# zju3dv/LoG

Hardware: NVIDIA B200
Metric: gaussians_per_s_fwd_bwd (higher is better)
Workload: dtype f32

## Files before the change

log_b200/csrc/lgr_blend.cu:

```cuda
#include "lgr_common.cuh"
#include "lgr_prof.cuh"

namespace lgr {

constexpr int BLEND_THREADS = TILE_PIX;
#ifndef LGR_FWD_MIN_CTAS
#define LGR_FWD_MIN_CTAS 5
#endif
#ifndef LGR_BWD_MIN_CTAS
#define LGR_BWD_MIN_CTAS 4
#endif
constexpr int BATCH = 256;
constexpr unsigned FULL = 0xffffffffu;

struct SubTile {
  int x, y;
  bool inside;
};

__device__ __forceinline__ SubTile make_subtile(const View& v, int tile, int lane, int warp) {
  SubTile s;
  const int tx = tile % v.gx, ty = v.row0 + tile / v.gx;
  const int sx = tx * TILE + (warp & 1) * 8, sy = ty * TILE + (warp >> 1) * 4;
  s.x = sx + (lane & 7); s.y = sy + (lane >> 3);
  s.inside = s.x < v.W && s.y < v.H;
  return s;
}

__device__ __forceinline__ unsigned subtile_bits(const float4 r0, const float4 r1, float tx0, float ty0) {
  const float xlo = r0.x - r1.z, xhi = r0.x + r1.z, ylo = r0.y - r1.w, yhi = r0.y + r1.w;
  unsigned xm = 0u, m = 0u;
  if (xhi >= tx0 && xlo <= tx0 + 7.0f) xm |= 1u;
  if (xhi >= tx0 + 8.0f && xlo <= tx0 + 15.0f) xm |= 2u;
#pragma unroll
  for (int r = 0; r < 4; r++)
    if (yhi >= ty0 + 4.0f * r && ylo <= ty0 + 4.0f * r + 3.0f) m |= xm << (2 * r);
  return m;
}

__device__ __forceinline__ float eval_power2(const float4 r0, const float con_z, float dx, float dy) {
  const float q = __fmaf_rn(r0.z, __fmul_rn(dx, dx), __fmul_rn(con_z, __fmul_rn(dy, dy)));
  return __fmaf_rn(-0.5f, q, -__fmul_rn(r0.w, __fmul_rn(dx, dy)));
}
__device__ __forceinline__ float ex2_approx(float x) {
  float y;
  asm("ex2.approx.ftz.f32 %0, %1;" : "=f"(y) : "f"(x));
  return y;
}
__device__ __forceinline__ float eval_alpha(float opacity, float G) { return fminf(ALPHA_MAX, __fmul_rn(opacity, G)); }

__device__ __forceinline__ uint32_t smem_u32(const void* p) { return (uint32_t)__cvta_generic_to_shared(p); }
__device__ __forceinline__ float4 lds_f4(uint32_t addr) {
  float4 v;
  asm volatile("ld.shared.v4.f32 {%0, %1, %2, %3}, [%4];" : "=f"(v.x), "=f"(v.y), "=f"(v.z), "=f"(v.w) : "r"(addr));
  return v;
}
__device__ __forceinline__ float2 lds_f2(uint32_t addr) {
  float2 v;
  asm volatile("ld.shared.v2.f32 {%0, %1}, [%2];" : "=f"(v.x), "=f"(v.y) : "r"(addr));
  return v;
}
__device__ __forceinline__ uint32_t pin_reg(uint32_t v) {
  asm volatile("" : "+r"(v));
  return v;
}
__device__ __forceinline__ void red_shared_max_u32(uint32_t addr, unsigned v) {
  asm volatile("red.shared.max.u32 [%0], %1;" ::"r"(addr), "r"(v) : "memory");
}
__device__ __forceinline__ void red_shared_add_f32(uint32_t addr, float v) {
  asm volatile("red.shared.add.f32 [%0], %1;" ::"r"(addr), "f"(v) : "memory");
}
__device__ __forceinline__ void sts_f32(uint32_t addr, float v) {
  asm volatile("st.shared.f32 [%0], %1;" ::"r"(addr), "f"(v) : "memory");
}
__device__ __forceinline__ float rcp_approx(float x) {
  float y;
  asm("rcp.approx.ftz.f32 %0, %1;" : "=f"(y) : "f"(x));
  return y;
}
__device__ __forceinline__ void prefetch_l2(const float* p) {
  asm volatile("prefetch.global.L2 [%0];" ::"l"(p));
}
__device__ __forceinline__ float tf32_lo(float x) { return x - __uint_as_float(__float_as_uint(x) & 0xffffe000u); }
__device__ __forceinline__ void ldsm_x4(uint32_t addr, uint32_t& r0, uint32_t& r1, uint32_t& r2, uint32_t& r3) {
  asm volatile("ldmatrix.sync.aligned.m8n8.x4.shared.b16 {%0, %1, %2, %3}, [%4];"
               : "=r"(r0), "=r"(r1), "=r"(r2), "=r"(r3) : "r"(addr));
}
__device__ __forceinline__ void mma_tf32(float& d0, float& d1, float& d2, float& d3, uint32_t a0, uint32_t a1, uint32_t a2,
                                         uint32_t a3, uint32_t b0, uint32_t b1) {
  asm volatile("mma.sync.aligned.m16n8k8.row.col.f32.tf32.tf32.f32 {%0, %1, %2, %3}, {%4, %5, %6, %7}, {%8, %9}, {%0, %1, %2, %3};"
               : "+f"(d0), "+f"(d1), "+f"(d2), "+f"(d3) : "r"(a0), "r"(a1), "r"(a2), "r"(a3), "r"(b0), "r"(b1));
}

__device__ __forceinline__ void stage_splat(float4* s_rec, unsigned char* s_bits, int slot, const float* __restrict__ splat,
                                            int id, float tx0, float ty0, const uint8_t* __restrict__ recorded = nullptr) {
  const float* rec = splat + (int64_t)id * LGR_SPLAT_FLOATS;
  const float4 r0 = ldg4(rec), r1 = ldg4(rec + 4);
  float4 r2 = ldg4(rec + 8);
  r2.w = __int_as_float(id);
  s_rec[3 * slot] = r0; s_rec[3 * slot + 1] = r1; s_rec[3 * slot + 2] = r2;
  s_bits[slot] = recorded ? *recorded : (unsigned char)subtile_bits(r0, r1, tx0, ty0);
}

template <bool AUX, bool REC>
__global__ void __launch_bounds__(BLEND_THREADS, LGR_FWD_MIN_CTAS)
blend_fwd_kernel(View v, const int32_t* __restrict__ tile_start, const int32_t* __restrict__ sorted_ids,
                 const float* __restrict__ splat, float* __restrict__ image, float* __restrict__ final_T,
                 int32_t* __restrict__ n_contrib, int32_t* __restrict__ pid_pixel, float* __restrict__ pw_pixel,
                 unsigned* __restrict__ point_weight_bits, int32_t* __restrict__ point_count) {
  __shared__ float4 s_rec[BATCH * 3];
  __shared__ unsigned s_w[AUX ? BATCH : 1];
  __shared__ unsigned char s_bits[BATCH];
  __shared__ unsigned s_cb[REC ? (BLEND_THREADS / 32) * (BATCH / 32) : 1];
  const int tile = blockIdx.x, tid = threadIdx.x, lane = tid & 31, warp = tid >> 5;
  const SubTile st = make_subtile(v, tile, lane, warp);
  const float pxf = (float)st.x, pyf = (float)st.y;
  const float tx0 = (float)((tile % v.gx) * TILE), ty0 = (float)((v.row0 + tile / v.gx) * TILE);
  const int beg = tile_start[tile], len = tile_start[tile + 1] - beg;
  const uint32_t s_w_addr = smem_u32(s_w);
  const uint32_t s_rec_addr = pin_reg(smem_u32(s_rec));

  float T = 1.0f, C0 = 0.f, C1 = 0.f, C2 = 0.f, wmax = 0.f;
  int last = 0, wid = -1;
  int done = st.inside ? 0 : 1;
  int id_next = tid < len ? sorted_ids[beg + tid] : -1;

  int base = 0, cnt = min(BATCH, len);
  auto stage = [&]() {
    if (tid < cnt) stage_splat(s_rec, s_bits, tid, splat, id_next, tx0, ty0);
    else s_bits[tid] = 0;
    if (AUX) s_w[tid] = 0u;
    id_next = base + BATCH + tid < len ? sorted_ids[beg + base + BATCH + tid] : -1;
    if (id_next >= 0) prefetch_l2(splat + (int64_t)id_next * LGR_SPLAT_FLOATS);
  };
  if (len > 0) stage();
  while (base < len) {
    __syncthreads();
    if (REC) {
      if (lane < BATCH / 32) s_cb[warp * (BATCH / 32) + lane] = 0u;
      __syncwarp();
    }
    if (!__all_sync(FULL, done)) {
      for (int c0 = 0; c0 < cnt; c0 += 32) {
        const int e_l = c0 + lane;
        unsigned mask = __ballot_sync(FULL, (s_bits[e_l] >> warp) & 1u);
        unsigned own_w = 0u;
        unsigned took = 0u;
        while (mask) {
          const int jA = __ffs(mask) - 1;
          mask &= mask - 1;
          const bool two = mask != 0u;
          const int jB = two ? __ffs(mask) - 1 : jA;
          mask &= mask - 1;
          const uint32_t recA = s_rec_addr + 48u * (uint32_t)(c0 + jA), recB = s_rec_addr + 48u * (uint32_t)(c0 + jB);
          const float4 r0A = lds_f4(recA), r0B = lds_f4(recB);
          const float2 r1A = lds_f2(recA + 16u), r1B = lds_f2(recB + 16u);
          const float dxA = __fsub_rn(r0A.x, pxf), dyA = __fsub_rn(r0A.y, pyf);
          const float dxB = __fsub_rn(r0B.x, pxf), dyB = __fsub_rn(r0B.y, pyf);
          const float powerA = eval_power2(r0A, r1A.x, dxA, dyA), powerB = eval_power2(r0B, r1B.x, dxB, dyB);
          const float alphaA = eval_alpha(r1A.y, ex2_approx(powerA)), alphaB = eval_alpha(r1B.y, ex2_approx(powerB));
          float wA = 0.f, wB = 0.f;
          if (!done && powerA <= 0.0f && alphaA >= ALPHA_MIN) {
            const float test_T = __fmul_rn(T, __fsub_rn(1.0f, alphaA));
            if (test_T < T_STOP) done = 1;
            else {
              wA = alphaA * T;
              const float4 r2 = lds_f4(recA + 32u);
              C0 = fmaf(r2.x, wA, C0); C1 = fmaf(r2.y, wA, C1); C2 = fmaf(r2.z, wA, C2);
              T = test_T;
              last = base + c0 + jA + 1;
              if (AUX && wA > wmax) { wmax = wA; wid = __float_as_int(r2.w); }
            }
          }
          if (two && !done && powerB <= 0.0f && alphaB >= ALPHA_MIN) {
            const float test_T = __fmul_rn(T, __fsub_rn(1.0f, alphaB));
            if (test_T < T_STOP) done = 1;
            else {
              wB = alphaB * T;
              const float4 r2 = lds_f4(recB + 32u);
              C0 = fmaf(r2.x, wB, C0); C1 = fmaf(r2.y, wB, C1); C2 = fmaf(r2.z, wB, C2);
              T = test_T;
              last = base + c0 + jB + 1;
              if (AUX && wB > wmax) { wmax = wB; wid = __float_as_int(r2.w); }
            }
          }
          if (AUX) {
            const unsigned mA = __reduce_max_sync(FULL, __float_as_uint(wA));
            const unsigned mB = __reduce_max_sync(FULL, __float_as_uint(wB));
            if (lane == jA) own_w = mA;
            if (two && lane == jB) own_w = mB;
          } else if (REC) {
            if (__any_sync(FULL, wA != 0.f)) took |= 1u << jA;
            if (__any_sync(FULL, wB != 0.f)) took |= 1u << jB;
          }
        }
        if (AUX && REC) took = __ballot_sync(FULL, own_w != 0u);
        if (REC && lane == 0) s_cb[warp * (BATCH / 32) + (c0 >> 5)] = took;
        if (AUX && own_w) red_shared_max_u32(s_w_addr + 4u * e_l, own_w);
        if (__all_sync(FULL, done)) break;
      }
    }
    const int all_done = __syncthreads_and(done);
    if (AUX && tid < cnt && s_w[tid]) atomicMax(point_weight_bits + __float_as_int(s_rec[3 * tid + 2].w), s_w[tid]);
    if (REC && tid < cnt) {
      unsigned byte = 0u;
#pragma unroll
      for (int w = 0; w < BLEND_THREADS / 32; w++) byte |= ((s_cb[w * (BATCH / 32) + (tid >> 5)] >> (tid & 31)) & 1u) << w;
      v.contrib[beg + base + tid] = (uint8_t)byte;
    }
    base += BATCH;
    if (all_done || base >= len) break;
    cnt = min(BATCH, len - base);
    stage();
  }
  if (st.inside) {
    const int64_t pix = (int64_t)st.y * v.W + st.x, HW = (int64_t)v.H * v.W;
    image[pix] = C0 + T * __ldg(v.bg);
    image[HW + pix] = C1 + T * __ldg(v.bg + 1);
    image[2 * HW + pix] = C2 + T * __ldg(v.bg + 2);
    final_T[pix] = T;
    n_contrib[pix] = last;
    if (AUX) {
      pid_pixel[pix] = (v.pid_map && wid >= 0) ? v.pid_map[wid] : wid; pw_pixel[pix] = wmax;
      if (point_count && wid >= 0) atomicAdd(point_count + wid, 1);
    }
  }
}

constexpr int HITS = 8;
constexpr int XROW = 36;
constexpr int BWD_SMEM = BATCH * 48 + BATCH * 36 + (BLEND_THREADS / 32) * (2 * HITS * XROW + 192 + 192) * 4 + BATCH;

template <bool REC>
__global__ void __launch_bounds__(BLEND_THREADS, LGR_BWD_MIN_CTAS)
blend_bwd_kernel(View v, const int32_t* __restrict__ tile_start, const int32_t* __restrict__ sorted_ids,
                 const float* __restrict__ splat, const float* __restrict__ image,
                 const float* __restrict__ dL_dimage, float* __restrict__ dsplat) {
  extern __shared__ float4 smem_f4[];
  float4* s_rec = smem_f4;
  float* s_g = reinterpret_cast<float*>(s_rec + BATCH * 3);
  float* s_x = s_g + BATCH * 9;
  float* s_cw = s_x + (BLEND_THREADS / 32) * 2 * HITS * XROW;
  float* s_mw = s_cw + (BLEND_THREADS / 32) * 192;
  unsigned char* s_bits = reinterpret_cast<unsigned char*>(s_mw + (BLEND_THREADS / 32) * 192);
  const int tile = blockIdx.x, tid = threadIdx.x, lane = tid & 31, warp = tid >> 5;
  const SubTile st = make_subtile(v, tile, lane, warp);
  const float pxf = (float)st.x, pyf = (float)st.y;
  const float tx0 = (float)((tile % v.gx) * TILE), ty0 = (float)((v.row0 + tile / v.gx) * TILE);
  const int beg = tile_start[tile], len = tile_start[tile + 1] - beg;
  const uint32_t s_g_addr = pin_reg(smem_u32(s_g));
  const uint32_t s_rec_addr = pin_reg(smem_u32(s_rec));
  const uint32_t xg_addr = pin_reg(smem_u32(s_x) + (uint32_t)warp * (2 * HITS * XROW * 4));
  const uint32_t xlane_addr = pin_reg(xg_addr + 4u * (uint32_t)lane);
  const uint32_t xrow = pin_reg(xg_addr + (uint32_t)(lane & 7) * (XROW * 4) + (uint32_t)((lane >> 3) & 1) * (HITS * XROW * 4) +
                                (uint32_t)(lane >> 4) * 16u);
  const float tcx = tx0 + 7.5f, tcy = ty0 + 7.5f;
  const int g = lane >> 2, t = lane & 3;

  float Rd = 0.f, dp0 = 0.f, dp1 = 0.f, dp2 = 0.f;
  int last = 0;
  if (st.inside) {
    const int64_t pix = (int64_t)st.y * v.W + st.x, HW = (int64_t)v.H * v.W;
    dp0 = dL_dimage[pix]; dp1 = dL_dimage[HW + pix]; dp2 = dL_dimage[2 * HW + pix];
    Rd = image[pix] * dp0 + image[HW + pix] * dp1 + image[2 * HW + pix] * dp2;
    if (REC) last = v.last_contrib[pix];
  }
  const uint32_t mw_addr = pin_reg(smem_u32(s_mw) + (uint32_t)warp * (192 * 4) + (uint32_t)((min(g, 5) * 4 + t) * 32));
  for (int k = lane; k < 192; k += 32) {
    const int which = k & 1, s_ = (k >> 1) & 3, t_ = (k >> 3) & 3, g_ = k >> 5;
    const float u = (float)((warp & 1) * 8 + t_ + 4 * which) - 7.5f, vv = (float)((warp >> 1) * 4 + s_) - 7.5f;
    const float f = g_ == 0 ? 1.f : g_ == 1 ? u : g_ == 2 ? vv : g_ == 3 ? u * u : g_ == 4 ? u * vv : vv * vv;
    s_mw[warp * 192 + k] = f;
  }
  const uint32_t cw_addr = pin_reg(smem_u32(s_cw) + (uint32_t)warp * (192 * 4) + (uint32_t)((min(g, 2) * 4 + t) * 64));
  {
    float* cw = s_cw + warp * 192;
    const int col = lane & 7, s = lane >> 3, tt = col & 3, which = col >> 2;
    const float dpc[3] = {dp0, dp1, dp2};
#pragma unroll
    for (int c = 0; c < 3; c++) {
      cw[((c * 4 + tt) * 4 + s) * 4 + which] = dpc[c];
      cw[((c * 4 + tt) * 4 + s) * 4 + 2 + which] = tf32_lo(dpc[c]);
    }
  }
  __syncwarp();

  float T = 1.0f;
  int done = st.inside ? (REC ? (last == 0) : 0) : 1;
  int id_next = tid < len ? sorted_ids[beg + tid] : -1;

  int base = 0, cnt = min(BATCH, len);
  auto stage = [&]() {
    if (tid < cnt) {
      stage_splat(s_rec, s_bits, tid, splat, id_next, tx0, ty0, REC ? v.contrib + beg + base + tid : nullptr);
#pragma unroll
      for (int k = 0; k < 9; k++) s_g[tid * 9 + k] = 0.f;
    } else {
      s_bits[tid] = 0;
    }
    id_next = base + BATCH + tid < len ? sorted_ids[beg + base + BATCH + tid] : -1;
    if (id_next >= 0) prefetch_l2(splat + (int64_t)id_next * LGR_SPLAT_FLOATS);
  };
  if (len > 0) stage();
  while (base < len) {
    __syncthreads();
    if (!__all_sync(FULL, done)) {
      int c0 = -32, pend = 0, my_e = 0;
      unsigned mask = 0u;
      bool fin = false;
      while (true) {
        if (mask == 0u) {
          do {
            c0 += 32;
            fin = c0 >= cnt || __all_sync(FULL, done);
            if (fin) break;
            mask = __ballot_sync(FULL, (s_bits[c0 + lane] >> warp) & 1u);
          } while (mask == 0u);
        }
        if (!fin) {
          const int jA = __ffs(mask) - 1;
          mask &= mask - 1;
          const bool two = mask != 0u;
          const int jB = two ? __ffs(mask) - 1 : jA;
          mask &= mask - 1;
          const int eA = c0 + jA, eB = c0 + jB;
          const uint32_t recA = s_rec_addr + 48u * (uint32_t)eA, recB = s_rec_addr + 48u * (uint32_t)eB;
          const float4 r0A = lds_f4(recA), r0B = lds_f4(recB);
          const float2 r1A = lds_f2(recA + 16u), r1B = lds_f2(recB + 16u);
          const float dxA = __fsub_rn(r0A.x, pxf), dyA = __fsub_rn(r0A.y, pyf);
          const float dxB = __fsub_rn(r0B.x, pxf), dyB = __fsub_rn(r0B.y, pyf);
          const float powerA = eval_power2(r0A, r1A.x, dxA, dyA), powerB = eval_power2(r0B, r1B.x, dxB, dyB);
          const float GA = ex2_approx(powerA), GB = ex2_approx(powerB);
          const float alphaA = eval_alpha(r1A.y, GA), alphaB = eval_alpha(r1B.y, GB);
          const float omA = __fsub_rn(1.0f, alphaA), omB = __fsub_rn(1.0f, alphaB);
          bool cA = false, cB = false;
          const float TA = T;
          float TB;
          if (REC) {
            cA = !done && powerA <= 0.0f && alphaA >= ALPHA_MIN;
            if (cA) T = __fmul_rn(T, omA);
            done = (base + eA + 1 >= last);
            TB = T;
            cB = two && !done && powerB <= 0.0f && alphaB >= ALPHA_MIN;
            if (cB) T = __fmul_rn(T, omB);
            if (two) done = (base + eB + 1 >= last);
          } else {
            if (!done && powerA <= 0.0f && alphaA >= ALPHA_MIN) {
              const float tt = __fmul_rn(T, omA);
              if (tt < T_STOP) done = 1; else { cA = true; T = tt; }
            }
            TB = T;
            if (two && !done && powerB <= 0.0f && alphaB >= ALPHA_MIN) {
              const float tt = __fmul_rn(T, omB);
              if (tt < T_STOP) done = 1; else { cB = true; T = tt; }
            }
          }
          const bool anyA = __any_sync(FULL, cA), anyB = __any_sync(FULL, cB);
          if (anyA) {
            float wG = 0.f, w = 0.f;
            if (cA) {
              const float4 r2 = lds_f4(recA + 32u);
              w = alphaA * TA;
              const float cdot = r2.x * dp0 + r2.y * dp1 + r2.z * dp2;
              Rd = fmaf(-cdot, w, Rd);
              const float dL_dalpha = cdot * TA - Rd * rcp_approx(omA);
              wG = r1A.y * dL_dalpha * GA;
            }
            const uint32_t row = xlane_addr + (uint32_t)pend * (XROW * 4);
            sts_f32(row, wG); sts_f32(row + HITS * XROW * 4, w);
            if (lane == pend) my_e = eA;
            pend++;
          }
          if (anyB) {
            float wG = 0.f, w = 0.f;
            if (cB) {
              const float4 r2 = lds_f4(recB + 32u);
              w = alphaB * TB;
              const float cdot = r2.x * dp0 + r2.y * dp1 + r2.z * dp2;
              Rd = fmaf(-cdot, w, Rd);
              const float dL_dalpha = cdot * TB - Rd * rcp_approx(omB);
              wG = r1B.y * dL_dalpha * GB;
            }
            const uint32_t row = xlane_addr + (uint32_t)pend * (XROW * 4);
            sts_f32(row, wG); sts_f32(row + HITS * XROW * 4, w);
            if (lane == pend) my_e = eB;
            pend++;
          }
        }
        if (pend >= HITS - 1 || (fin && pend > 0)) {
          __syncwarp();
          float d0 = 0.f, d1 = 0.f, z0 = 0.f, z1 = 0.f, y0 = 0.f, y1 = 0.f, d2 = 0.f, d3 = 0.f;
#pragma unroll
          for (int s = 0; s < 4; s++) {
            uint32_t a0, a1, a2, a3;
            ldsm_x4(xrow + 32u * s, a0, a1, a2, a3);
            const uint32_t l0 = __float_as_uint(tf32_lo(__uint_as_float(a0))), l1 = __float_as_uint(tf32_lo(__uint_as_float(a1)));
            const uint32_t l2 = __float_as_uint(tf32_lo(__uint_as_float(a2))), l3 = __float_as_uint(tf32_lo(__uint_as_float(a3)));
            float2 bm = make_float2(0.f, 0.f);
            float4 bc = make_float4(0.f, 0.f, 0.f, 0.f);
            if (g < 6) bm = lds_f2(mw_addr + 8u * s);
            if (g < 3) bc = lds_f4(cw_addr + 16u * s);
            mma_tf32(d0, d1, z0, z1, a0, a1, a2, a3, __float_as_uint(bm.x), __float_as_uint(bm.y));
            mma_tf32(y0, y1, d2, d3, a0, a1, a2, a3, __float_as_uint(bc.x), __float_as_uint(bc.y));
            mma_tf32(d0, d1, z0, z1, l0, l1, l2, l3, __float_as_uint(bm.x), __float_as_uint(bm.y));
            mma_tf32(y0, y1, d2, d3, l0, l1, l2, l3, __float_as_uint(bc.x), __float_as_uint(bc.y));
            mma_tf32(y0, y1, d2, d3, a0, a1, a2, a3, __float_as_uint(bc.z), __float_as_uint(bc.w));
          }
          const uint32_t acc = s_g_addr + 36u * (uint32_t)__shfl_sync(FULL, my_e, g);
          if (g < pend) {
            if (t < 3) { red_shared_add_f32(acc + 8u * t, d0); red_shared_add_f32(acc + 8u * t + 4u, d1); }
            if (t < 2) red_shared_add_f32(acc + 24u + 8u * t, d2);
            if (t == 0) red_shared_add_f32(acc + 28u, d3);
          }
          __syncwarp();
          pend = 0;
        }
        if (fin) break;
      }
    }
    const int all_done = __syncthreads_and(done);
    if (tid < cnt) {
      const float* m = s_g + tid * 9;
      const float M00 = m[0], M10 = m[1], M01 = m[2], M20 = m[3], M11 = m[4], M02 = m[5];
      const bool nz = (M00 != 0.f) | (M10 != 0.f) | (M01 != 0.f) | (M20 != 0.f) | (M11 != 0.f) | (M02 != 0.f) |
                      (m[6] != 0.f) | (m[7] != 0.f) | (m[8] != 0.f);
      if (nz) {
        const float4 r0 = s_rec[3 * tid];
        const float2 r1 = *reinterpret_cast<const float2*>(&s_rec[3 * tid + 1]);
        const int id = __float_as_int(s_rec[3 * tid + 2].w);
        const float X = r0.x - tcx, Y = r0.y - tcy;
        const float Sx = fmaf(X, M00, -M10), Sy = fmaf(Y, M00, -M01);
        const float Sxx = fmaf(X, fmaf(X, M00, -2.f * M10), M20);
        const float Syy = fmaf(Y, fmaf(Y, M00, -2.f * M01), M02);
        const float Sxy = fmaf(X, fmaf(Y, M00, -M01), fmaf(-Y, M10, M11));
        float4 a, b;
        a.x = -(r0.z * Sx + r0.w * Sy);
        a.y = -(r1.x * Sy + r0.w * Sx);
        a.z = -0.5f * Sxx;
        a.w = -Sxy;
        b.x = -0.5f * Syy;
        b.y = M00 / r1.y;
        b.z = m[6]; b.w = m[7];
        float4* dst = reinterpret_cast<float4*>(dsplat + (int64_t)id * LGR_GRAD_FLOATS);
        atomicAdd(dst, a);
        atomicAdd(dst + 1, b);
        atomicAdd(reinterpret_cast<float*>(dst + 2), m[8]);
      }
    }
    base += BATCH;
    if (all_done || base >= len) break;
    cnt = min(BATCH, len - base);
    stage();
  }
}

int launch_blend_fwd(const View& v, const int32_t* tile_start, const int32_t* sorted_ids, const float* splat,
                     float* image, float* final_T, int32_t* n_contrib, int32_t* pid_pixel, float* pw_pixel,
                     float* point_weight, int32_t* point_count, cudaStream_t st) {
  const int ntiles = v.gx * (v.row1 - v.row0);
  if (ntiles <= 0) return 0;
  ProfScope ps(K_BLEND_FWD, st);
  unsigned* pwb = reinterpret_cast<unsigned*>(point_weight);
  const bool rec = v.contrib != nullptr;
  if (v.want_aux && rec)
    blend_fwd_kernel<true, true><<<ntiles, BLEND_THREADS, 0, st>>>(v, tile_start, sorted_ids, splat, image, final_T, n_contrib, pid_pixel, pw_pixel, pwb, point_count);
  else if (v.want_aux)
    blend_fwd_kernel<true, false><<<ntiles, BLEND_THREADS, 0, st>>>(v, tile_start, sorted_ids, splat, image, final_T, n_contrib, pid_pixel, pw_pixel, pwb, point_count);
  else if (rec)
    blend_fwd_kernel<false, true><<<ntiles, BLEND_THREADS, 0, st>>>(v, tile_start, sorted_ids, splat, image, final_T, n_contrib, pid_pixel, pw_pixel, pwb, point_count);
  else
    blend_fwd_kernel<false, false><<<ntiles, BLEND_THREADS, 0, st>>>(v, tile_start, sorted_ids, splat, image, final_T, n_contrib, pid_pixel, pw_pixel, pwb, point_count);
  LGR_CHECK_LAUNCH();
  return 0;
}

int launch_blend_bwd(const View& v, const int32_t* tile_start, const int32_t* sorted_ids, const float* splat,
                     const float* image, const float* dL_dimage, float* dsplat, cudaStream_t st) {
  const int ntiles = v.gx * (v.row1 - v.row0);
  if (ntiles <= 0) return 0;
  const bool rec = v.contrib != nullptr && v.last_contrib != nullptr;
  cudaError_t e = rec ? cudaFuncSetAttribute(blend_bwd_kernel<true>, cudaFuncAttributeMaxDynamicSharedMemorySize, BWD_SMEM)
                      : cudaFuncSetAttribute(blend_bwd_kernel<false>, cudaFuncAttributeMaxDynamicSharedMemorySize, BWD_SMEM);
  if (e != cudaSuccess) return (int)e;
  ProfScope ps(K_BLEND_BWD, st);
  if (rec) blend_bwd_kernel<true><<<ntiles, BLEND_THREADS, BWD_SMEM, st>>>(v, tile_start, sorted_ids, splat, image, dL_dimage, dsplat);
  else blend_bwd_kernel<false><<<ntiles, BLEND_THREADS, BWD_SMEM, st>>>(v, tile_start, sorted_ids, splat, image, dL_dimage, dsplat);
  LGR_CHECK_LAUNCH();
  return 0;
}

}
```

profiles/sass_census.py:

```python
import collections
import os
import re
import subprocess

ROOT = os.path.dirname(os.path.dirname(os.path.abspath(__file__)))
LIB = os.path.join(ROOT, 'log_b200', '_lib', 'liblog_b200_raster.so')
PATS = collections.OrderedDict([
    ('HMMA (mma.sync tf32)', r'\bHMMA\.'), ('LDSM (ldmatrix)', r'\bLDSM'), ('UTC*MMA / LDTM (tcgen05)', r'UTC\w*MMA|LDTM'),
    ('UBLKCP / UTMA (bulk / tensor copies)', r'UBLKCP|UTMA'), ('REDUX', r'\bREDUX'), ('VOTE', r'\bVOTE'), ('MATCH', r'\bMATCH'),
    ('SHFL', r'\bSHFL'), ('ATOMS / REDS (shared)', r'\bATOMS|\bREDS'), ('ATOMG (returning)', r'\bATOMG'), ('RED (global)', r'\bRED\.'),
    ('MUFU.EX2', r'MUFU\.EX2'), ('BAR', r'\bBAR\.'), ('LDG.128', r'LDG\.E\.(\w+\.)*128'), ('STG.128', r'STG\.E\.(\w+\.)*128'),
    ('CCTL (L2 prefetch)', r'\bCCTL')])


def main():
    sass = subprocess.run(['cuobjdump', '-sass', LIB], capture_output=True, text=True, check=True).stdout
    stats, cur = collections.OrderedDict(), None
    for line in sass.splitlines():
        m = re.search(r'Function : (\S+)', line)
        if m:
            cur = m.group(1)
            stats[cur] = collections.Counter()
        elif cur and re.search(r'/\*[0-9a-f]{4}\*/', line):
            stats[cur]['instructions'] += 1
            for k, p in PATS.items():
                if re.search(p, line):
                    stats[cur][k] += 1
    print('# SASS census of `liblog_b200_raster.so` (sm_100a), static instruction counts per kernel\n')
    print('`cuobjdump -sass` of the shipped library, grouped by `profiles/sass_census.py`. The tensor-core path is the legacy')
    print('`mma.sync.m16n8k8.tf32` (`HMMA.1688.F32.TF32`) fed by `ldmatrix` (`LDSM`) in `blend_bwd_kernel`; there is no')
    print('`tcgen05` / TMA instruction in the library (the path has no GEMM-shaped stage large enough to own TMEM, DESIGN.md §3).\n')
    print('| kernel | instructions | ' + ' | '.join(PATS) + ' |')
    print('|---|---|' + '---|' * len(PATS))
    for k, c in stats.items():
        name = subprocess.run(['c++filt', k], capture_output=True, text=True).stdout.strip().split('(')[0].replace('void ', '').replace('lgr::', '')
        print(f'| `{name}` | {c["instructions"]} | ' + ' | '.join(str(c[p]) if c[p] else '' for p in PATS) + ' |')


if __name__ == '__main__':
    main()
```

Before: 2.325 billion.

## Flush per-warp MMA moments straight to global atomics, drop shared accumulator

The backward blend kernel no longer accumulates per-splat moment sums in a shared s_g buffer through shared-memory float reductions followed by a per-batch epilogue. Each warp now rearranges its MMA outputs with shuffles, computes the gradient parts in place, and issues vector float4 global atomicAdds per hit group. The moment weights are recentred on each warp's subtile centre and the B-operand layouts are reindexed so that every lane reads unconditionally. Dropping s_g shrinks shared memory under 48KB, which removes the opt-in call and may raise occupancy. The trade-off is far more global atomics, one per warp hit rather than one per splat per tile, which increases contention and L2 traffic.

```diff
diff --git a/log_b200/csrc/lgr_blend.cu b/log_b200/csrc/lgr_blend.cu
--- a/log_b200/csrc/lgr_blend.cu
+++ b/log_b200/csrc/lgr_blend.cu
@@ -66,9 +66,6 @@
 }
 __device__ __forceinline__ void red_shared_max_u32(uint32_t addr, unsigned v) {
   asm volatile("red.shared.max.u32 [%0], %1;" ::"r"(addr), "r"(v) : "memory");
-}
-__device__ __forceinline__ void red_shared_add_f32(uint32_t addr, float v) {
-  asm volatile("red.shared.add.f32 [%0], %1;" ::"r"(addr), "f"(v) : "memory");
 }
 __device__ __forceinline__ void sts_f32(uint32_t addr, float v) {
   asm volatile("st.shared.f32 [%0], %1;" ::"r"(addr), "f"(v) : "memory");
@@ -229,7 +226,8 @@
 
 constexpr int HITS = 8;
 constexpr int XROW = 36;
-constexpr int BWD_SMEM = BATCH * 48 + BATCH * 36 + (BLEND_THREADS / 32) * (2 * HITS * XROW + 192 + 192) * 4 + BATCH;
+constexpr int BWD_SMEM = BATCH * 48 + (BLEND_THREADS / 32) * (2 * HITS * XROW + 192 + 192) * 4 + BATCH;
+static_assert(BWD_SMEM <= 48 * 1024, "the backward launches without the large-shared-memory opt-in");
 
 template <bool REC>
 __global__ void __launch_bounds__(BLEND_THREADS, LGR_BWD_MIN_CTAS)
@@ -238,8 +236,7 @@
                  const float* __restrict__ dL_dimage, float* __restrict__ dsplat) {
   extern __shared__ float4 smem_f4[];
   float4* s_rec = smem_f4;
-  float* s_g = reinterpret_cast<float*>(s_rec + BATCH * 3);
-  float* s_x = s_g + BATCH * 9;
+  float* s_x = reinterpret_cast<float*>(s_rec + BATCH * 3);
   float* s_cw = s_x + (BLEND_THREADS / 32) * 2 * HITS * XROW;
   float* s_mw = s_cw + (BLEND_THREADS / 32) * 192;
   unsigned char* s_bits = reinterpret_cast<unsigned char*>(s_mw + (BLEND_THREADS / 32) * 192);
@@ -248,13 +245,13 @@
   const float pxf = (float)st.x, pyf = (float)st.y;
   const float tx0 = (float)((tile % v.gx) * TILE), ty0 = (float)((v.row0 + tile / v.gx) * TILE);
   const int beg = tile_start[tile], len = tile_start[tile + 1] - beg;
-  const uint32_t s_g_addr = pin_reg(smem_u32(s_g));
   const uint32_t s_rec_addr = pin_reg(smem_u32(s_rec));
   const uint32_t xg_addr = pin_reg(smem_u32(s_x) + (uint32_t)warp * (2 * HITS * XROW * 4));
   const uint32_t xlane_addr = pin_reg(xg_addr + 4u * (uint32_t)lane);
   const uint32_t xrow = pin_reg(xg_addr + (uint32_t)(lane & 7) * (XROW * 4) + (uint32_t)((lane >> 3) & 1) * (HITS * XROW * 4) +
                                 (uint32_t)(lane >> 4) * 16u);
-  const float tcx = tx0 + 7.5f, tcy = ty0 + 7.5f;
+  const float ucx = (warp & 1) * 8 + 3.5f, ucy = (warp >> 1) * 4 + 1.5f;
+  const float tcx = tx0 + ucx, tcy = ty0 + ucy;
   const int g = lane >> 2, t = lane & 3;
 
   float Rd = 0.f, dp0 = 0.f, dp1 = 0.f, dp2 = 0.f;
@@ -265,22 +262,22 @@
     Rd = image[pix] * dp0 + image[HW + pix] * dp1 + image[2 * HW + pix] * dp2;
     if (REC) last = v.last_contrib[pix];
   }
-  const uint32_t mw_addr = pin_reg(smem_u32(s_mw) + (uint32_t)warp * (192 * 4) + (uint32_t)((min(g, 5) * 4 + t) * 32));
+  const uint32_t mw_addr = pin_reg(smem_u32(s_mw) + (uint32_t)warp * (192 * 4) + (uint32_t)min(lane, 23) * 8u);
   for (int k = lane; k < 192; k += 32) {
-    const int which = k & 1, s_ = (k >> 1) & 3, t_ = (k >> 3) & 3, g_ = k >> 5;
-    const float u = (float)((warp & 1) * 8 + t_ + 4 * which) - 7.5f, vv = (float)((warp >> 1) * 4 + s_) - 7.5f;
+    const int which = k & 1, s_ = (k >> 1) / 24, l_ = (k >> 1) % 24, t_ = l_ & 3, g_ = l_ >> 2;
+    const float u = (float)((warp & 1) * 8 + t_ + 4 * which) - ucx, vv = (float)((warp >> 1) * 4 + s_) - ucy;
     const float f = g_ == 0 ? 1.f : g_ == 1 ? u : g_ == 2 ? vv : g_ == 3 ? u * u : g_ == 4 ? u * vv : vv * vv;
     s_mw[warp * 192 + k] = f;
   }
-  const uint32_t cw_addr = pin_reg(smem_u32(s_cw) + (uint32_t)warp * (192 * 4) + (uint32_t)((min(g, 2) * 4 + t) * 64));
+  const uint32_t cw_addr = pin_reg(smem_u32(s_cw) + (uint32_t)warp * (192 * 4) + (uint32_t)min(lane, 11) * 16u);
   {
     float* cw = s_cw + warp * 192;
     const int col = lane & 7, s = lane >> 3, tt = col & 3, which = col >> 2;
     const float dpc[3] = {dp0, dp1, dp2};
 #pragma unroll
     for (int c = 0; c < 3; c++) {
-      cw[((c * 4 + tt) * 4 + s) * 4 + which] = dpc[c];
-      cw[((c * 4 + tt) * 4 + s) * 4 + 2 + which] = tf32_lo(dpc[c]);
+      cw[(s * 12 + c * 4 + tt) * 4 + which] = dpc[c];
+      cw[(s * 12 + c * 4 + tt) * 4 + 2 + which] = tf32_lo(dpc[c]);
     }
   }
   __syncwarp();
@@ -293,8 +290,6 @@
   auto stage = [&]() {
     if (tid < cnt) {
       stage_splat(s_rec, s_bits, tid, splat, id_next, tx0, ty0, REC ? v.contrib + beg + base + tid : nullptr);
-#pragma unroll
-      for (int k = 0; k < 9; k++) s_g[tid * 9 + k] = 0.f;
     } else {
       s_bits[tid] = 0;
     }
@@ -396,21 +391,45 @@
             ldsm_x4(xrow + 32u * s, a0, a1, a2, a3);
             const uint32_t l0 = __float_as_uint(tf32_lo(__uint_as_float(a0))), l1 = __float_as_uint(tf32_lo(__uint_as_float(a1)));
             const uint32_t l2 = __float_as_uint(tf32_lo(__uint_as_float(a2))), l3 = __float_as_uint(tf32_lo(__uint_as_float(a3)));
-            float2 bm = make_float2(0.f, 0.f);
-            float4 bc = make_float4(0.f, 0.f, 0.f, 0.f);
-            if (g < 6) bm = lds_f2(mw_addr + 8u * s);
-            if (g < 3) bc = lds_f4(cw_addr + 16u * s);
+            const float2 bm = lds_f2(mw_addr + 192u * s);
+            const float4 bc = lds_f4(cw_addr + 192u * s);
             mma_tf32(d0, d1, z0, z1, a0, a1, a2, a3, __float_as_uint(bm.x), __float_as_uint(bm.y));
             mma_tf32(y0, y1, d2, d3, a0, a1, a2, a3, __float_as_uint(bc.x), __float_as_uint(bc.y));
             mma_tf32(d0, d1, z0, z1, l0, l1, l2, l3, __float_as_uint(bm.x), __float_as_uint(bm.y));
             mma_tf32(y0, y1, d2, d3, l0, l1, l2, l3, __float_as_uint(bc.x), __float_as_uint(bc.y));
             mma_tf32(y0, y1, d2, d3, a0, a1, a2, a3, __float_as_uint(bc.z), __float_as_uint(bc.w));
           }
-          const uint32_t acc = s_g_addr + 36u * (uint32_t)__shfl_sync(FULL, my_e, g);
-          if (g < pend) {
-            if (t < 3) { red_shared_add_f32(acc + 8u * t, d0); red_shared_add_f32(acc + 8u * t + 4u, d1); }
-            if (t < 2) red_shared_add_f32(acc + 24u + 8u * t, d2);
-            if (t == 0) red_shared_add_f32(acc + 28u, d3);
+          const int e = __shfl_sync(FULL, my_e, g);
+          const int src = (lane & ~3) | ((0x3102 >> (4 * t)) & 3);
+          const float x0 = __shfl_xor_sync(FULL, d0, 1);
+          const float x1 = __shfl_down_sync(FULL, d1, 1);
+          const float x2 = __shfl_sync(FULL, t == 2 ? d0 : d2, src);
+          const float x3 = __shfl_xor_sync(FULL, d3, 1);
+          if (g < pend && t < 3) {
+            const uint32_t rec = s_rec_addr + 48u * (uint32_t)e;
+            const float4 r0 = lds_f4(rec);
+            const float2 r1 = lds_f2(rec + 16u);
+            float* dst = dsplat + (int64_t)__float_as_int(lds_f2(rec + 40u).y) * LGR_GRAD_FLOATS;
+            const float X = r0.x - tcx, Y = r0.y - tcy;
+            float4 part;
+            if (t == 0) {
+              const float M00 = d0, M10 = d1, M01 = x0, M20 = x1, M11 = x2;
+              const float Sx = fmaf(X, M00, -M10), Sy = fmaf(Y, M00, -M01);
+              const float Sxx = fmaf(X, fmaf(X, M00, -2.f * M10), M20);
+              const float Sxy = fmaf(X, fmaf(Y, M00, -M01), fmaf(-Y, M10, M11));
+              part.x = -(r0.z * Sx + r0.w * Sy);
+              part.y = -(r1.x * Sy + r0.w * Sx);
+              part.z = -0.5f * Sxx;
+              part.w = -Sxy;
+            } else if (t == 1) {
+              const float M00 = x0, M01 = d0, M02 = x1;
+              part.x = -0.5f * fmaf(Y, fmaf(Y, M00, -2.f * M01), M02);
+              part.y = M00 * rcp_approx(r1.y);
+              part.z = x2; part.w = x3;
+            } else {
+              part = make_float4(x2, 0.f, 0.f, 0.f);
+            }
+            atomicAdd(reinterpret_cast<float4*>(dst) + t, part);
           }
           __syncwarp();
           pend = 0;
@@ -419,34 +438,6 @@
       }
     }
     const int all_done = __syncthreads_and(done);
-    if (tid < cnt) {
-      const float* m = s_g + tid * 9;
-      const float M00 = m[0], M10 = m[1], M01 = m[2], M20 = m[3], M11 = m[4], M02 = m[5];
-      const bool nz = (M00 != 0.f) | (M10 != 0.f) | (M01 != 0.f) | (M20 != 0.f) | (M11 != 0.f) | (M02 != 0.f) |
-                      (m[6] != 0.f) | (m[7] != 0.f) | (m[8] != 0.f);
-      if (nz) {
-        const float4 r0 = s_rec[3 * tid];
-        const float2 r1 = *reinterpret_cast<const float2*>(&s_rec[3 * tid + 1]);
-        const int id = __float_as_int(s_rec[3 * tid + 2].w);
-        const float X = r0.x - tcx, Y = r0.y - tcy;
-        const float Sx = fmaf(X, M00, -M10), Sy = fmaf(Y, M00, -M01);
-        const float Sxx = fmaf(X, fmaf(X, M00, -2.f * M10), M20);
-        const float Syy = fmaf(Y, fmaf(Y, M00, -2.f * M01), M02);
-        const float Sxy = fmaf(X, fmaf(Y, M00, -M01), fmaf(-Y, M10, M11));
-        float4 a, b;
-        a.x = -(r0.z * Sx + r0.w * Sy);
-        a.y = -(r1.x * Sy + r0.w * Sx);
-        a.z = -0.5f * Sxx;
-        a.w = -Sxy;
-        b.x = -0.5f * Syy;
-        b.y = M00 / r1.y;
-        b.z = m[6]; b.w = m[7];
-        float4* dst = reinterpret_cast<float4*>(dsplat + (int64_t)id * LGR_GRAD_FLOATS);
-        atomicAdd(dst, a);
-        atomicAdd(dst + 1, b);
-        atomicAdd(reinterpret_cast<float*>(dst + 2), m[8]);
-      }
-    }
     base += BATCH;
     if (all_done || base >= len) break;
     cnt = min(BATCH, len - base);
@@ -479,9 +470,6 @@
   const int ntiles = v.gx * (v.row1 - v.row0);
   if (ntiles <= 0) return 0;
   const bool rec = v.contrib != nullptr && v.last_contrib != nullptr;
-  cudaError_t e = rec ? cudaFuncSetAttribute(blend_bwd_kernel<true>, cudaFuncAttributeMaxDynamicSharedMemorySize, BWD_SMEM)
-                      : cudaFuncSetAttribute(blend_bwd_kernel<false>, cudaFuncAttributeMaxDynamicSharedMemorySize, BWD_SMEM);
-  if (e != cudaSuccess) return (int)e;
   ProfScope ps(K_BLEND_BWD, st);
   if (rec) blend_bwd_kernel<true><<<ntiles, BLEND_THREADS, BWD_SMEM, st>>>(v, tile_start, sorted_ids, splat, image, dL_dimage, dsplat);
   else blend_bwd_kernel<false><<<ntiles, BLEND_THREADS, BWD_SMEM, st>>>(v, tile_start, sorted_ids, splat, image, dL_dimage, dsplat);
diff --git a/profiles/r03_ab_table.py b/profiles/r03_ab_table.py
--- /dev/null
+++ b/profiles/r03_ab_table.py
@@ -0,0 +1,35 @@
+import collections
+import glob
+import json
+import os
+import re
+import sys
+
+
+def main(out):
+    runs = collections.defaultdict(list)
+    for f in sorted(glob.glob(os.path.join(out, 'bench_*_*_*.json'))):
+        m = re.match(r'bench_(\w+?)_(old|new|sg)_(\d+)\.json', os.path.basename(f))
+        lines = [ln for ln in open(f).read().splitlines() if ln.startswith('{')]
+        if not m or not lines:
+            print(f'{os.path.basename(f)}: no result line')
+            continue
+        d = json.loads(lines[-1])
+        runs[(m.group(1), m.group(2))].append((int(m.group(3)), d['ms_per_step'], d['kernel_ms']['blend_bwd'],
+                                               d.get('clocks', {}).get('sm_mhz')))
+    print('| workload | library | run | ms_per_step | blend_bwd ms | SM MHz |')
+    print('|---|---|---|---|---|---|')
+    for (w, v), rs in sorted(runs.items()):
+        for rep, ms, bwd, mhz in sorted(rs):
+            print(f'| {w} | {v} | {rep} | {ms:.4f} | {bwd:.4f} | {mhz} |')
+    print('\n| workload | library | runs | ms_per_step median (spread) | blend_bwd median (spread) |')
+    print('|---|---|---|---|---|')
+    for (w, v), rs in sorted(runs.items()):
+        ms = sorted(r[1] for r in rs)
+        bwd = sorted(r[2] for r in rs)
+        print(f'| {w} | {v} | {len(rs)} | {ms[len(ms) // 2]:.4f} ({ms[-1] - ms[0]:.4f}) | '
+              f'{bwd[len(bwd) // 2]:.4f} ({bwd[-1] - bwd[0]:.4f}) |')
+
+
+if __name__ == '__main__':
+    main(sys.argv[1])
diff --git a/profiles/r03_compare_dumps.py b/profiles/r03_compare_dumps.py
--- /dev/null
+++ b/profiles/r03_compare_dumps.py
@@ -0,0 +1,30 @@
+import os
+import sys
+
+import numpy as np
+
+FORWARD = ('gaussian_index', 'pixel_index', 'image', 'radii', 'point_id_pixel', 'point_weight_pixel', 'point_weight')
+
+
+def main(old_dir, new_dir):
+    names = sorted(f[:-4] for f in os.listdir(old_dir) if f.endswith('.npy'))
+    assert names == sorted(f[:-4] for f in os.listdir(new_dir) if f.endswith('.npy')), 'different file sets'
+    bad = False
+    for name in names:
+        a = np.load(os.path.join(old_dir, name + '.npy')).astype(np.float64)
+        b = np.load(os.path.join(new_dir, name + '.npy')).astype(np.float64)
+        same = a.shape == b.shape and np.array_equal(a, b, equal_nan=True)
+        rel = float(np.linalg.norm(b - a) / max(np.linalg.norm(a), 1e-300)) if a.shape == b.shape else float('inf')
+        if name in FORWARD:
+            verdict = 'bit-identical' if same else 'DIFFERS'
+            bad |= not same
+        else:
+            verdict = 'ok' if rel <= 1e-5 else 'ABOVE 1e-5'
+            bad |= rel > 1e-5
+        print(f'{name:22s} shape={str(a.shape):14s} bit-identical={same!s:5s} rel={rel:.3e}  {verdict}')
+    print('RESULT:', 'FAIL' if bad else 'PASS')
+    return 1 if bad else 0
+
+
+if __name__ == '__main__':
+    sys.exit(main(sys.argv[1], sys.argv[2]))
diff --git a/profiles/sass_census.py b/profiles/sass_census.py
--- a/profiles/sass_census.py
+++ b/profiles/sass_census.py
@@ -8,7 +8,7 @@
 PATS = collections.OrderedDict([
     ('HMMA (mma.sync tf32)', r'\bHMMA\.'), ('LDSM (ldmatrix)', r'\bLDSM'), ('UTC*MMA / LDTM (tcgen05)', r'UTC\w*MMA|LDTM'),
     ('UBLKCP / UTMA (bulk / tensor copies)', r'UBLKCP|UTMA'), ('REDUX', r'\bREDUX'), ('VOTE', r'\bVOTE'), ('MATCH', r'\bMATCH'),
-    ('SHFL', r'\bSHFL'), ('ATOMS / REDS (shared)', r'\bATOMS|\bREDS'), ('ATOMG (returning)', r'\bATOMG'), ('RED (global)', r'\bRED\.'),
+    ('SHFL', r'\bSHFL'), ('ATOMS / REDS (shared)', r'\bATOMS|\bREDS'), ('ATOMG (returning)', r'\bATOMG'), ('RED (global)', r'\bREDG?\.E\.'),
     ('MUFU.EX2', r'MUFU\.EX2'), ('BAR', r'\bBAR\.'), ('LDG.128', r'LDG\.E\.(\w+\.)*128'), ('STG.128', r'STG\.E\.(\w+\.)*128'),
     ('CCTL (L2 prefetch)', r'\bCCTL')])
 
```

Result: faster. 2.452 billion (median of 6 runs) (+5.5%).
